# Wubeizhongxinghua/BSSeqConsensusReads

Measured on AMD Instinct MI355X. Metric: duplex families/sec (node) at 1/2/4/8 MI355X; % HBM roofline; speedup vs CPU, higher is better.
Workload: dtype int64 fixed-point log-likelihood sums (2^-20 nats) + fp32 exp; fp64 read-order sums on near ties; u8 nt16 bases / phred quals; 1 GPU; C2 -- configs[1]: 1M-family synthetic WGBS grouped BAM, 2x150bp, Poisson(4) family size, one MI355X; families_per_gpu=1000000, consensus_families_per_gpu=1151121, batches_per_gpu=1, family_order=fgbio TemplateCoordinate runs of one MI, records_per_gpu=8150056, bases_per_gpu=1222508400, small_families=1151121, large_families=0, parallelism=family-sharded x1

## Files before the change

bsseqconsensusreads_amd/csrc/bsdc_kernels.hip:

```cpp
#include <hip/hip_runtime.h>

#include <algorithm>
#include <cmath>
#include <cstdio>
#include <cstdlib>
#include <cstring>
#include <string>

#include "../../include/bsdc.h"
#include "../../include/bsdc_layout.h"

namespace {

constexpr int kWave = 64;
#ifndef SMALL_STAGE_U
#define SMALL_STAGE_U 4
#endif
constexpr int kStageU = SMALL_STAGE_U;
#ifndef LARGE_THREADS
#define LARGE_THREADS 256
#endif
constexpr int kLargeThreads = LARGE_THREADS;
#ifndef LARGE_THREADS_BIG
#define LARGE_THREADS_BIG 512
// ... 566 lines not shown
    }
}
struct OvlDw {
    Ovl4 in;
    uint32_t A0, inm;
    int32_t B0;
    int lo, hi;
};
__device__ __forceinline__ OvlDw ovl_dw_load(const uint8_t *bimg, const uint8_t *qimg, uint32_t xa, uint32_t xb, int ovl,
                                            int d) {
    OvlDw t;
    const int p0 = 4 * d - (int)(xa & 3u);
    t.A0 = (xa & ~3u) + 4u * (uint32_t)d;
    t.B0 = (int32_t)xb + p0;
    t.lo = ::max(-p0, 0);
    t.hi = ::min(ovl - p0, 4);
    t.inm = t.hi > t.lo ? (0xFFFFFFFFu >> (32 - 8 * (t.hi - t.lo))) << (8 * t.lo) : 0u;
    if (t.hi > t.lo) {
        const int32_t Bl = t.B0 + t.lo;
        const uint32_t sh = 8u * (uint32_t)t.lo;
        t.in = Ovl4{lds32(bimg + t.A0), lds_any32(bimg, Bl) << sh, lds32(qimg + t.A0), lds_any32(qimg, Bl) << sh};
    }
    return t;
}
__device__ __forceinline__ void ovl_dw_store(uint8_t *bimg, uint8_t *qimg, const OvlDw &t) {
    if (t.hi <= t.lo) return;
    const Ovl4 o = ovl4_compute_m(t.in, t.inm);
    const bool whole = t.inm == 0xFFFFFFFFu;
    st32(bimg + t.A0, o.x);
    st32(qimg + t.A0, o.qa);
    if (whole && (t.B0 & 3) == 0) {
        st32(bimg + t.B0, o.y);
        st32(qimg + t.B0, o.qb);
    } else if (whole) {
        stu32(bimg + t.B0, o.y);
        stu32(qimg + t.B0, o.qb);
    } else {
        for (int k = t.lo; k < t.hi; k++) {
            bimg[t.B0 + k] = (uint8_t)(o.y >> (8 * k));
            qimg[t.B0 + k] = (uint8_t)(o.qb >> (8 * k));
        }
    }
}
__device__ __forceinline__ void ovl4_store(uint8_t *bimg, uint8_t *qimg, uint32_t ia, uint32_t ib, int rem, const Ovl4 &o) {
    if (rem >= 4) {
        stu32(bimg + ia, o.x);
        stu32(bimg + ib, o.y);
        stu32(qimg + ia, o.qa);
        stu32(qimg + ib, o.qb);
    } else {
        for (int k = 0; k < rem; k++) {
            bimg[ia + k] = (uint8_t)(o.x >> (8 * k));
            bimg[ib + k] = (uint8_t)(o.y >> (8 * k));
            qimg[ia + k] = (uint8_t)(o.qa >> (8 * k));
            qimg[ib + k] = (uint8_t)(o.qb >> (8 * k));
        }
    }
}
__device__ __forceinline__ void overlap4(uint8_t *bimg, uint8_t *qimg, uint32_t ia, uint32_t ib, int rem) {
    ovl4_store(bimg, qimg, ia, ib, rem, ovl4_compute(ovl4_load(bimg, qimg, ia, ib), rem));
}
__device__ __forceinline__ void lookup4(const int32_t *lr2, uint32_t b, uint32_t q, int32_t &D0, int32_t &D1,
                                        int32_t &D2, int32_t &D3) {
    const uint32_t v = (b >> 4) & 0x01010101u;
    const uint32_t lo = __builtin_amdgcn_perm(v, q, 0x05010400u) << 2;
    const uint32_t hi = __builtin_amdgcn_perm(v, q, 0x07030602u) << 2;
    const uint8_t *base = reinterpret_cast<const uint8_t *>(lr2);
    D0 += *reinterpret_cast<const int32_t *>(base + (lo & 0xFFFFu));
    D1 += *reinterpret_cast<const int32_t *>(base + (lo >> 16));
    D2 += *reinterpret_cast<const int32_t *>(base + (hi & 0xFFFFu));
    D3 += *reinterpret_cast<const int32_t *>(base + (hi >> 16));
}
__device__ __forceinline__ void lookup4v(const int32_t *lr2, uint32_t v, uint32_t q, int32_t &D0, int32_t &D1,
                                         int32_t &D2, int32_t &D3) {
    const uint32_t lo = __builtin_amdgcn_perm(v, q, 0x05010400u) << 2;
    const uint32_t hi = __builtin_amdgcn_perm(v, q, 0x07030602u) << 2;
    const uint8_t *base = reinterpret_cast<const uint8_t *>(lr2);
    D0 += *reinterpret_cast<const int32_t *>(base + (lo & 0xFFFFu));
    D1 += *reinterpret_cast<const int32_t *>(base + (lo >> 16));
    D2 += *reinterpret_cast<const int32_t *>(base + (hi & 0xFFFFu));
    D3 += *reinterpret_cast<const int32_t *>(base + (hi >> 16));
}
__device__ __forceinline__ uint32_t onehot01(uint32_t x) {
    const uint32_t r = __builtin_amdgcn_perm(0x00000001u, 0x00018100u, x);
    return r & ~((x + 0x03030303u) >> 4) & 0x01010101u;
}
__device__ __forceinline__ uint32_t bytes_past(int k8, bool reverse) {
    const uint32_t s = (uint32_t)::min(::max(k8, 0), 32);
    return reverse ? (uint32_t)(0xFFFFFFFFull >> s) : (uint32_t)(~0ull << s);
}
__device__ __forceinline__ uint32_t expand80(uint32_t m80) { return m80 | (m80 - (m80 >> 7)); }
__device__ __forceinline__ uint32_t bytes_nonzero(uint32_t x) {
    return expand80((x + 0x7F7F7F7Fu) & 0x80808080u);
}
__device__ __forceinline__ void resolve4(bool ha, bool hb, uint32_t bmA, uint32_t QA, uint32_t bmB, uint32_t QB,
                                         uint32_t qadd, uint32_t &ob, uint32_t &oq, uint32_t *ss) {
    const uint32_t okA = expand80((QA + qadd) & 0x80808080u);
    const uint32_t okB = expand80((QB + qadd) & 0x80808080u);
    const uint32_t bA = (bmA & okA) | (0x0F0F0F0Fu & ~okA), qA = (QA & okA) | (0x02020202u & ~okA);
    const uint32_t bB = (bmB & okB) | (0x0F0F0F0Fu & ~okB), qB = (QB & okB) | (0x02020202u & ~okB);
    ss[0] = bA;
    ss[1] = qA;
    ss[2] = bB;
    ss[3] = qB;
    if (!(ha && hb)) {
        ob = ha ? bA : bB;
        oq = ha ? qA : qB;
        return;
    }
    const uint32_t same = ~bytes_nonzero(bA ^ bB);
    const uint32_t dAB = (qA | 0x80808080u) - qB;
    const uint32_t geA = expand80(dAB & 0x80808080u);
    const uint32_t dBA = (qB | 0x80808080u) - qA;
    const uint32_t ad = ((dAB & geA) | (dBA & ~geA)) & 0x7F7F7F7Fu;
    const uint32_t sum = qA + qB;
    const uint32_t over = expand80((sum + 0x22222222u) & 0x80808080u);
    const uint32_t sum93 = (sum & ~over) | (0x5D5D5D5Du & over);
    const uint32_t ad2 = ad | (0x02020202u & ~bytes_nonzero(ad));
    uint32_t rb = (bA & (same | geA)) | (bB & ~(same | geA));
    uint32_t rq = (sum93 & same) | (ad2 & ~same);
    const uint32_t isN = ((bA + 0x01010101u) | (bB + 0x01010101u)) & 0x10101010u;
    const uint32_t is2 = ~bytes_nonzero(rq ^ 0x02020202u);
    const uint32_t nm = expand80(isN << 3) | is2;
    ob = (rb & ~nm) | (0x0F0F0F0Fu & nm);
    oq = (rq & ~nm) | (0x02020202u & nm);
}
__device__ __forceinline__ uint32_t comp4(uint32_t x) {
    return (__builtin_bitreverse32(__builtin_bswap32(x)) >> 4) & 0x0F0F0F0Fu;
}
template <bool FLAG>
__device__ __forceinline__ void unpack32(uint4 v, uint8_t *dst) {
    const uint32_t w[4] = {v.x, v.y, v.z, v.w};
    uint32_t o[8];
#pragma unroll
    for (int k = 0; k < 4; k++) {
        uint32_t lo = w[k] & 0x0F0F0F0Fu;
        uint32_t hi = (w[k] >> 4) & 0x0F0F0F0Fu;
        if (FLAG) {
            const uint32_t a = w[k], b = w[k] >> 1, c = w[k] >> 2, d = w[k] >> 3;
            const uint32_t ab = a | b, cd = c | d;
            const uint32_t two = (a & b) | (c & d) | (ab & cd);
            const uint32_t vm = (ab | cd) & ~two & 0x11111111u;
            lo |= (vm << 4) & 0x10101010u;
            hi |= vm & 0x10101010u;
        }
        o[2 * k] = __builtin_amdgcn_perm(lo, hi, 0x05010400u);
        o[2 * k + 1] = __builtin_amdgcn_perm(lo, hi, 0x07030602u);
    }
    uint4 *d = reinterpret_cast<uint4 *>(dst);
    d[0] = make_uint4(o[0], o[1], o[2], o[3]);
    d[1] = make_uint4(o[4], o[5], o[6], o[7]);
}

template <bool TAGS>
__device__ __forceinline__ void small_family(const KParams &P, const Tables *T, uint8_t *A, const uint32_t *fams,
                                             int64_t fi, int t) {
    const int32_t *lr2 = T->zero;
    const float *thr = T->thr;
    const uint8_t *qlo = T->qlo;
    const int32_t *dthr = T->dthr;
    const bsdc_family_batch &B = P.B;
    const bool do_convert = P.mode & BSDC_MODE_CONVERT;
    const bool do_extend = P.mode & BSDC_MODE_EXTEND;
    const bool do_vote = P.mode & BSDC_MODE_VOTE;
    const int max_len = B.max_len;
    const int stop = (P.mode >> BSDC_MODE_STOP_SHIFT) & 15;

    const uint4 ent = reinterpret_cast<const uint4 *>(fams)[__builtin_amdgcn_readfirstlane((int)fi)];
    const uint32_t fam = __builtin_amdgcn_readfirstlane(ent.x);
    const uint32_t r0 = __builtin_amdgcn_readfirstlane(ent.y);
    const int n = (int)(__builtin_amdgcn_readfirstlane(ent.z) & 0xFF);
    const uint32_t img = (__builtin_amdgcn_readfirstlane(ent.z) >> 8) * 32u;
    const uint32_t base_g = __builtin_amdgcn_readfirstlane(ent.w);

    const bool has = t < n;
    uint4 rc = make_uint4(0, 0, 0, 0);
    uint2 win = make_uint2(0, 0);
    uint32_t cinfo = 0;
    if (has) {
        rc = reinterpret_cast<const uint4 *>(B.rec)[r0 + t];
        win = reinterpret_cast<const uint2 *>(B.rec_win)[r0 + t];
        cinfo = B.cig_info[r0 + t];
    }
    const int nqc = (int)(img >> 4), nch = nqc + (int)(img >> 5);
    uint8_t *bimg = A;
    uint8_t *qimg = A + img;
    uint32_t qor = 0;
    for (int u = 0; u < ((nqc + 63) >> 6); u++) {
        const int k = t + 64 * u;
        if (k < nqc) glds16(B.qual + base_g + 16u * (uint32_t)k, qimg + 1024 * u);
    }
    auto load_img = [&](int k) {
        uint4 v = make_uint4(0, 0, 0, 0);
        if (k < nch) v = *reinterpret_cast<const uint4 *>(B.seq + (base_g >> 1) + 16 * (uint32_t)(k - nqc));
        return v;
    };
    auto store_img = [&](int k, uint4 v) {
        if (k < nch) unpack32<true>(v, bimg + 32 * (k - nqc));
    };
    auto kmap = [&](int u) {
        const int kb = t + 64 * u;
        return kb < nch - nqc ? nqc + kb : nch;
    };
    uint4 v[kStageU];
#pragma unroll
    for (int u = 0; u < kStageU; u++) v[u] = load_img(kmap(u));

    const uint32_t gslot = rc.x;
    int32_t pos = (int32_t)rc.y;
    const int32_t L = (int32_t)(rc.z & 0xFFFF);
    const uint32_t flag = rc.z >> 16;
    uint32_t link = rc.w;
    const bool conv = has && do_convert && (link & BSDC_LINK_CONVERT);
    const bool cplx = has && (link & BSDC_LINK_COMPLEX);
    if (!cplx) cinfo = 0;
    const uint64_t conv_mask = ballot(conv);
    const int nconv = __builtin_popcountll(conv_mask);
    const int ci = mbcnt(conv_mask);
    int cops = (int)(cinfo & 0xFFFF);
    if (ballot(cops != 0)) {
#pragma unroll
        for (int o = 32; o >= 1; o >>= 1) cops += __shfl_xor(cops, o, kWave);
    }
    const SmallLayout Lo(n, img, nconv, cops, max_len);
    uint8_t *refw = A + Lo.ref;
    const int ws = Lo.ws;
    uint32_t *lc = reinterpret_cast<uint32_t *>(A + Lo.misc);
    uint8_t *convlane = A + Lo.misc + 16;
    uint32_t *convwin = reinterpret_cast<uint32_t *>(A + Lo.lists);
    const uint32_t slot = gslot - base_g;
    if (conv) {
        convwin[ci] = win.x;
        convlane[ci] = (uint8_t)t;
    }
    if (t < 4) lc[t] = 0;
    wave_sync();
    const uint32_t rcn = (uint32_t)P.ref_chunks, rinv = P.ref_chunks_inv;
    const int wtot = nconv * (int)rcn;
    auto load_win = [&](int k) {
        uint4 x = make_uint4(0, 0, 0, 0);
        if (k < wtot) {
            const uint32_t cr = __umulhi((uint32_t)k, rinv), part = (uint32_t)k - cr * rcn;
            x = *reinterpret_cast<const uint4 *>(P.ref + ((convwin[cr] >> 1) & ~15u) + 16 * part);
        }
        return x;
    };
    auto store_win = [&](int k, uint4 x) {
        if (k < wtot) {
            const uint32_t cr = __umulhi((uint32_t)k, rinv), part = (uint32_t)k - cr * rcn;
            unpack32<false>(x, refw + cr * ws + 32 * part);
        }
    };
    uint4 wv[2];
#pragma unroll
    for (int u = 0; u < 2; u++) wv[u] = load_win(t + 64 * u);
    __builtin_amdgcn_s_setprio(0);
#pragma unroll
    for (int u = 0; u < kStageU; u++) store_img(kmap(u), v[u]);
    const int ub = (nch - nqc + 63) >> 6;
    for (int u0 = kStageU; u0 < ub; u0 += kStageU) {
#pragma unroll
        for (int u = 0; u < kStageU; u++) v[u] = load_img(kmap(u0 + u));
#pragma unroll
        for (int u = 0; u < kStageU; u++) store_img(kmap(u0 + u), v[u]);
    }
#pragma unroll
    for (int u = 0; u < 2; u++) store_win(t + 64 * u, wv[u]);
    for (int k0 = 128; k0 < wtot; k0 += 128) {
#pragma unroll
        for (int u = 0; u < 2; u++) wv[u] = load_win(k0 + t + 64 * u);
#pragma unroll
        for (int u = 0; u < 2; u++) store_win(k0 + t + 64 * u, wv[u]);
    }
    __asm__ volatile("s_waitcnt vmcnt(0)" ::: "memory");
    wave_sync();
    for (int k = t; k < nqc; k += 64) {
        const uint4 q = *reinterpret_cast<const uint4 *>(qimg + 16 * k);
        qor |= q.x | q.y | q.z | q.w;
    }
    wave_sync();
    if (stop == 1) return;

    int32_t start = 1, len = L;
    bool rd = false;
    for (int cr0 = 0; cr0 < nconv; cr0 += 4) {
        const int cr = cr0 + (t >> 4);
        const bool act = cr < nconv;
        const int src = act ? convlane[cr] : 0;
        const uint32_t s_slot = (uint32_t)__shfl((int)slot, src, kWave);
        const int32_t s_L = __shfl(L, src, kWave);
        const uint32_t s_win = (uint32_t)__shfl((int)win.x, src, kWave);
        const int32_t s_avail = __shfl((int)win.y, src, kWave);
        bool my_rd = false;
        if (act) {
            const int32_t Lm = s_L + 1;
            const uint32_t wbase = (uint32_t)(cr * ws) + (s_win & 31u);
            for (int j4 = 4 * (t & 15); j4 < Lm; j4 += 64) {
                uint32_t m = lds32(bimg + s_slot + j4);
                const uint32_t mn = lds32(bimg + s_slot + j4 + 4);
                const uint32_t a = wbase + (uint32_t)j4;
                const uint32_t d0 = lds32(refw + (a & ~3u)), d1 = lds32(refw + (a & ~3u) + 4);
                const uint32_t sh = a & 3u;
                uint32_t f0 = alignbyte(d1, d0, sh);
                uint32_t f1 = sh == 3 ? d1 : alignbyte(d1, d0, sh + 1);
                if (j4 + 5 > s_avail) {
#pragma unroll
                    for (int k = 0; k < 4; k++) {
                        if (j4 + k >= s_avail) f0 = (f0 & ~(0xFFu << (8 * k))) | (kN << (8 * k));
                        if (j4 + k + 1 >= s_avail) f1 = (f1 & ~(0xFFu << (8 * k))) | (kN << (8 * k));
                    }
                }
                if (j4 == 0) {
                    const uint32_t r0b = f0 & 0xFFu;
                    m = (m & ~0xFFu) | r0b | ((r0b != 0 && (r0b & (r0b - 1)) == 0) ? 0x10u : 0u);
                }
                const uint32_t m1 = alignbyte(mn, m, 1);
                uint32_t nxt = 0x80808080u;
                const int last = Lm - 1 - j4;
                if (last >= 0 && last < 4) nxt &= ~(0xFFu << (8 * last));
                const uint32_t out = convert4f(m, m1, f0, f1, nxt);
                st32(bimg + s_slot + j4, out);
                if (last >= 0 && last < 4)
                    my_rd = ((out >> (8 * last)) & 0x0F) == kC && ((f1 >> (8 * last)) & 0x0F) == kG;
            }
            if ((t & 15) == 0) qimg[s_slot] = 40;
        }
        const uint64_t bal = ballot(my_rd);
        if (conv && (ci >> 2) == (cr0 >> 2) && ((bal >> (16 * (ci & 3))) & 0xFFFFu)) rd = true;
    }
    if (conv) {
        start = 0;
        len = L + 1 - (rd ? 1 : 0);
        pos = pos - 1 > 0 ? pos - 1 : 0;
    }
    if (!do_convert && has && (link & BSDC_LINK_RD_IN)) rd = true;
    if (rd) link |= kLinkRdDev;
    wave_sync();
    if (stop == 2) return;

    if (do_extend) {
        const int p = (int)((link >> BSDC_LINK_PARTNER_SHIFT) & 3u);
        const uint32_t p_slot = (uint32_t)__shfl((int)slot, p, kWave);
        const int32_t p_start = __shfl(start, p, kWave);
        const int32_t p_len = __shfl(len, p, kWave);
        const bool er = has && (link & BSDC_LINK_EXT_RIGHT);
        const bool el = has && (link & BSDC_LINK_EXT_LEFT) && rd;
        uint32_t b0 = 0, q0 = 0, bl = 0, ql = 0;
        if (er) {
            b0 = bimg[p_slot + p_start];
            q0 = qimg[p_slot + p_start];
        }
        if (el) {
            if (p_len > 0) {
                bl = bimg[p_slot + p_start + p_len - 1];
                ql = qimg[p_slot + p_start + p_len - 1];
            } else {
                bl = bimg[slot + start];
                ql = qimg[slot + start];
            }
        }
        if (er) {
            bimg[slot + start - 1] = (uint8_t)b0;
            qimg[slot + start - 1] = (uint8_t)q0;
            start -= 1;
            len += 1;
            pos -= 1;
        }
        if (el) {
            bimg[slot + start + len] = (uint8_t)bl;
            qimg[slot + start + len] = (uint8_t)ql;
            len += 1;
        }
        wave_sync();
    }

    int32_t reflen = len;
    if (cplx) {
        reflen = (int32_t)(cinfo >> 16) + (conv ? 1 : 0) - ((conv && rd) ? 1 : 0) +
                 ((do_extend && (link & BSDC_LINK_EXT_RIGHT)) ? 1 : 0) +
                 ((do_extend && (link & BSDC_LINK_EXT_LEFT) && rd) ? 1 : 0);
    }

    if (P.mode & BSDC_MODE_DUMP) {
        for (int r = 0; r < n; r++) {
            const uint32_t s_slot = rlu(slot, r), s_g = rlu(gslot, r);
            const int32_t s_start = rl(start, r), s_len = rl(len, r);
            for (int j = t; j < s_len; j += 64) {
                P.O.dump_seq[s_g + j] = bimg[s_slot + s_start + j] & 0x0F;
                P.O.dump_qual[s_g + j] = qimg[s_slot + s_start + j];
            }
        }
        if (has) {
            const uint32_t gi = r0 + t;
            P.O.dump_pos[gi] = pos;
            P.O.dump_len[gi] = (uint16_t)len;
            uint8_t tg = 0;
            if (rd) tg |= 1;
            if (conv) tg |= 2 | 4;
            if (do_extend && (link & BSDC_LINK_EXT_RIGHT)) tg |= 4;
            if (do_extend && (link & BSDC_LINK_EXT_LEFT) && rd) tg |= 8;
            P.O.dump_tags[gi] = tg;
        }
    }
    if (!do_vote || stop == 3) return;

// ... 250 lines not shown
                        const uint32_t q0 = qlo[d >> 16];
                        Qp[side] |= (q0 + (d >= dthr[q0 + 1] ? 1u : 0u)) << (8 * j);
                    }
                }
                uint32_t ob4, oq4, ss[4];
                resolve4(hA, hB, bm[0], Qp[0], bm[1], Qp[1], qadd, ob4, oq4, ss);
                const uint32_t inA = TAGS ? ~bytes_past(8 * (la - c), false) : ~0u;
                const uint32_t inB = TAGS ? ~bytes_past(8 * (lb - c), false) : ~0u;
                const uint32_t slowA = hA ? (bytes_nonzero(multi[0] & 0x7F7F7F7Fu) | negm[0]) & inA : 0u;
                const uint32_t slowB = hB ? (bytes_nonzero(multi[1] & 0x7F7F7F7Fu) | negm[1]) & inB : 0u;
                const uint32_t slow4 = (slowA | slowB) & ~bytes_past(8 * (lv - c), false);
                if (slow4) {
                    const uint32_t useA = hA ? ~slowA : 0u, useB = (hB ? ~slowB : 0u) & ~useA;
                    const uint32_t fb = (ss[0] & useA) | ((ss[2] | 0x10101010u) & useB);
                    const uint32_t fq = (ss[1] & useA) | (ss[3] & useB);
                    ob4 = (ob4 & ~slow4) | (fb & slow4);
                    oq4 = (oq4 & ~slow4) | (fq & slow4);
                }
#pragma unroll
                for (int j = 0; j < 4; j++) {
                    const bool qd = ((slow4 >> (8 * j)) & 0xFFu) != 0;
                    const uint64_t ms = ballot(qd);
                    if (ms == 0) continue;
                    if (qd) sq[nq + mbcnt(ms)] = (uint16_t)((e << 15) | (c + j));
                    nq += __builtin_popcountll(ms);
                }
                if (c < lv) {
                    st32(outb + e * ow + c, ob4);
                    st32(outq + e * ow + c, oq4);
                }
                if (TAGS && c < lv) {
#pragma unroll
                    for (int side = 0; side < 2; side++) {
                        const int s = side == 0 ? sa : sb;
                        if (!(side == 0 ? hA : hB)) continue;
                        const uint32_t n4 = nf[side] + __builtin_bswap32(nr[side]);
                        const int64_t at = (4 * (int64_t)fam + s) * stride + c;
                        *reinterpret_cast<uint32_t *>(P.O.ss_base + at) = ss[2 * side];
                        *reinterpret_cast<uint32_t *>(P.O.ss_qual + at) = ss[2 * side + 1];
                        *reinterpret_cast<uint32_t *>(P.O.ss_depth + at) = n4;
                        *reinterpret_cast<uint32_t *>(P.O.ss_err + at) = 0u;
                    }
                }
            }
        }
        wave_sync();
        if (stop == 7) nq = 0;
        const uint32_t hsm = (hs[0] ? 1u : 0u) | (hs[1] ? 2u : 0u) | (hs[2] ? 4u : 0u) | (hs[3] ? 8u : 0u);
        const int side = t & 1;
        for (int k0 = 0; k0 < 2 * nq && stop != 9; k0 += 64) {
            const int k = (k0 + t) >> 1;
            const bool act = k < nq;
            const uint32_t ent = act ? sq[k] : 0u;
            const int e = (int)(ent >> 15), c = (int)(ent & 0x7FFF);
            const int s = side == 0 ? e : 3 - e;
            const int ns = s == 0 ? cnt[0] : s == 1 ? cnt[1] : s == 2 ? cnt[2] : cnt[3];
            const int os = s == 0 ? off[0] : s == 1 ? off[1] : s == 2 ? off[2] : off[3];
            const bool have = act && ((hsm >> s) & 1u);
            const uint32_t kb = act ? outb[e * ow + c] : 0u, kq = act ? outq[e * ow + c] : 0u;
            uint32_t vb = 0, vq = 0;
            if (have && kq != 0 && (int)((kb >> 4) & 1) == side) {
                vb = kb & 0x0F;
                vq = kq;
            } else if (have) {
                int32_t D0 = 0, D1 = 0, D2 = 0, D3 = 0;
                uint32_t n0 = 0, n1 = 0, n2 = 0, n3 = 0;
                uint32_t seen = 0;
                for (int i = 0; i < ns; i++) {
                    const uint32_t d = dlist[os + i];
                    if (c >= (int)((d >> 16) & 0x7FFF)) continue;
                    const uint32_t idx = (d & 0x80000000u) ? (d & 0xFFFF) - c : (d & 0xFFFF) + c;
                    const uint32_t braw = bimg[idx];
                    seen |= braw;
                    const int32_t v = lr2[(braw >> 4) * 256u + qimg[idx]];
                    const uint32_t bb = (d & 0x80000000u) ? comp_nt16(braw) : (braw & 0x0F);
                    D0 += bb == kA ? v : 0;
                    D1 += bb == kC ? v : 0;
                    D2 += bb == kG ? v : 0;
                    D3 += bb == kT ? v : 0;
                    if (TAGS) {
                        n0 += bb == kA ? 1u : 0u;
                        n1 += bb == kC ? 1u : 0u;
                        n2 += bb == kG ? 1u : 0u;
                        n3 += bb == kT ? 1u : 0u;
                    }
                }
                int best = first_max4(D0, D1, D2, D3);
                if (near_tie(D0, D1, D2, D3, best, ns))
                    best = fp64_pick(SmallDesc{dlist + os}, ns, c, bimg, qimg, P.tab->lnc, P.tab->lne3);
                const SsCall sc = ss_call(D0, D1, D2, D3, best, (seen & 0x10u) != 0, n0, n1, n2, n3, thr, P.qmin);
                vb = sc.base;
                vq = sc.qual;
                if (TAGS) {
                    const int64_t at = (4 * (int64_t)fam + s) * stride + c;
                    P.O.ss_base[at] = (uint8_t)vb;
                    P.O.ss_qual[at] = (uint8_t)vq;
                    P.O.ss_depth[at] = (uint8_t)sc.depth;
                    P.O.ss_err[at] = (uint8_t)sc.err;
                }
            }
            const uint32_t pb = (uint32_t)__shfl_xor((int)vb, 1, kWave), pq = (uint32_t)__shfl_xor((int)vq, 1, kWave);
            if (act && side == 0) {
                const bool ha = (hsm >> e) & 1u, hb = (hsm >> (3 - e)) & 1u;
                uint32_t ob, oq;
                if (ha && hb) {
                    duplex_col(vb, vq, pb, pq, ob, oq);
                } else {
                    ob = ha ? vb : pb;
                    oq = ha ? vq : pq;
                }
                outb[e * ow + c] = (uint8_t)ob;
                outq[e * ow + c] = (uint8_t)oq;
            }
        }
        wave_sync();
        if (stop != 7 && stop != 8) {
            const int e = t >> 5;
            const int ol = e ? olen[1] : olen[0];
            for (int c0 = 8 * (t & 31); c0 < ol; c0 += 256) {
                uint2 bv = *reinterpret_cast<const uint2 *>(outb + e * ow + c0);
                uint2 qv = *reinterpret_cast<const uint2 *>(outq + e * ow + c0);
                const int k8 = 8 * (ol - c0);
                const uint32_t keep0 = ~bytes_past(k8, false), keep1 = ~bytes_past(k8 - 32, false);
                bv.x &= keep0;
                bv.y &= keep1;
                const uint32_t qlo2 = qv.x & keep0, qhi2 = qv.y & keep1;
                const uint32_t t0 = (bv.x << 4) | (bv.x >> 8), t1 = (bv.y << 4) | (bv.y >> 8);
                const uint32_t pk = __builtin_amdgcn_perm(t1, t0, 0x06040200u);
                const int64_t so = (2 * (int64_t)fam + e) * stride;
                *reinterpret_cast<uint32_t *>(P.O.seq + so / 2 + c0 / 2) = pk;
                *reinterpret_cast<uint2 *>(P.O.qual + so + c0) = make_uint2(qlo2, qhi2);
            }
        }
    }
    if (TAGS && t < 4) P.O.ss_len[4 * fam + t] = (uint16_t)(t == 0 ? (hs[0] ? lcs[0] : 0) : t == 1 ? (hs[1] ? lcs[1] : 0)
                                                             : t == 2 ? (hs[2] ? lcs[2] : 0) : (hs[3] ? lcs[3] : 0));
    if (t == 0) {
        uint8_t st = emit ? 1 : 0;
        if (hs[0] || hs[1]) st |= 2;
        if (hs[2] || hs[3]) st |= 4;
        P.O.status[fam] = st;
        P.O.len[2 * fam] = (uint16_t)(emit ? olen[0] : 0);
        P.O.len[2 * fam + 1] = (uint16_t)(emit ? olen[1] : 0);
    }
}

template <bool TAGS>
__global__ __launch_bounds__(kWave *kSmallMaxWaves, kSmallMinWaves) __attribute__((amdgpu_num_sgpr(96))) void k_small(
    KParams P, const uint32_t *fams, int64_t nfams, int32_t arena) {
    extern __shared__ __attribute__((aligned(16))) uint8_t smem[];
    __shared__ __attribute__((aligned(16))) Tables s_tab;
    if (((P.mode >> BSDC_MODE_STOP_SHIFT) & 15) == 15) return;
    __builtin_amdgcn_s_setprio(3);
    load_tables<kTabBytes>(&P.tab->t, reinterpret_cast<uint8_t *>(&s_tab));
    if (((P.mode >> BSDC_MODE_STOP_SHIFT) & 15) == 14) return;
    const int w = threadIdx.x >> 6;
    const int t = threadIdx.x & 63;
    const int64_t fi = (int64_t)blockIdx.x * (blockDim.x >> 6) + w;
    uint8_t *A = smem + kArenaGuard + (size_t)w * (size_t)arena;
    if (fi < nfams) small_family<TAGS>(P, &s_tab, A, fams, fi, t);
}

struct RecMeta {
    int32_t pos;
    int32_t len;
    uint32_t slot;
    int32_t avail;
    int32_t start;
    uint32_t link;
    uint32_t gidx;
    uint32_t win;
    int32_t srclen;
    int32_t reflen;
    uint16_t flag;
    uint8_t rd;
    uint8_t set;
    int32_t in_len;
};
static_assert(sizeof(RecMeta) == bsdc_layout::kRecMetaBytes, "RecMeta layout");


template <int G>
__device__ __forceinline__ int block_sum(int v, int *red) {
#pragma unroll
    for (int o = 32; o >= 1; o >>= 1) v += __shfl_xor(v, o, kWave);
    __syncthreads();
    if ((threadIdx.x & 63) == 0) red[threadIdx.x >> 6] = v;
    __syncthreads();
    int s = 0;
    for (int w = 0; w < G / kWave; w++) s += red[w];
    __syncthreads();
    return s;
}
template <int G>
__device__ __forceinline__ int block_max(int v, int *red) {
#pragma unroll
    for (int o = 32; o >= 1; o >>= 1) v = ::max(v, __shfl_xor(v, o, kWave));
    __syncthreads();
    if ((threadIdx.x & 63) == 0) red[threadIdx.x >> 6] = v;
    __syncthreads();
    int s = red[0];
    for (int w = 1; w < G / kWave; w++) s = ::max(s, red[w]);
    __syncthreads();
    return s;
}

template <int G>
__device__ __forceinline__ void block_sum_max(int a, int b, int *red, int &sum, int &mx) {
#pragma unroll
    for (int o = 32; o >= 1; o >>= 1) {
        a += __shfl_xor(a, o, kWave);
        b = ::max(b, __shfl_xor(b, o, kWave));
    }
    if ((threadIdx.x & 63) == 0) {
        red[threadIdx.x >> 6] = a;
        red[G / kWave + (threadIdx.x >> 6)] = b;
    }
    __syncthreads();
    sum = 0;
    mx = red[G / kWave];
    for (int w = 0; w < G / kWave; w++) {
        sum += red[w];
        mx = ::max(mx, red[G / kWave + w]);
    }
}

template <int G, bool TAGS>
__device__ void large_emit(const KParams &P, uint32_t fam, const int *cnt, const int *lcv, const uint8_t *ssb,
                           const uint8_t *ssq, int ssw, bool tag_rows) {
    const int tt = threadIdx.x;
    bool hs[4];
    for (int s = 0; s < 4; s++) hs[s] = cnt[s] > 0 && lcv[s] > 0;
    const bool emit = (hs[0] || hs[3]) && (hs[1] || hs[2]);
    const int32_t stride = P.O.stride;
    int olen[2];
    for (int e = 0; e < 2; e++) {
        const int sa = e == 0 ? 0 : 1, sb2 = e == 0 ? 3 : 2;
        olen[e] = (hs[sa] && hs[sb2]) ? ::min(lcv[sa], lcv[sb2]) : hs[sa] ? lcv[sa] : hs[sb2] ? lcv[sb2] : 0;
    }
    if (emit) {
        for (int e = 0; e < 2; e++) {
            const int sa = e == 0 ? 0 : 1, sb2 = e == 0 ? 3 : 2;
            const int64_t so = (2 * (int64_t)fam + e) * stride;
            const int npair = (olen[e] + 1) >> 1;
            for (int k = tt; k < npair; k += G) {
                uint32_t ob[2] = {0, 0}, oq[2] = {0, 0};
                for (int h = 0; h < 2; h++) {
                    const int col = 2 * k + h;
                    if (col >= olen[e]) break;
                    if (hs[sa] && hs[sb2]) {
                        duplex_col(ssb[sa * ssw + col], ssq[sa * ssw + col], ssb[sb2 * ssw + col], ssq[sb2 * ssw + col],
                                   ob[h], oq[h]);
                    } else {
                        const int s1 = hs[sa] ? sa : sb2;
                        ob[h] = ssb[s1 * ssw + col];
                        oq[h] = ssq[s1 * ssw + col];
                    }
                }
                P.O.seq[so / 2 + k] = (uint8_t)((ob[0] << 4) | ob[1]);
                P.O.qual[so + 2 * k] = (uint8_t)oq[0];
                if (2 * k + 1 < olen[e]) P.O.qual[so + 2 * k + 1] = (uint8_t)oq[1];
            }
        }
    }
    if (TAGS && tag_rows) {
        for (int s = 0; s < 4; s++) {
            const int ls = hs[s] ? lcv[s] : 0;
            const int64_t row = (4 * (int64_t)fam + s) * stride;
            for (int c = tt; c < ls; c += G) {
                P.O.ss_base[row + c] = ssb[s * ssw + c];
                P.O.ss_qual[row + c] = ssq[s * ssw + c];
            }
        }
        if (tt < 4) P.O.ss_len[4 * fam + tt] = (uint16_t)(hs[tt] ? lcv[tt] : 0);
    }
    if (tt == 0) {
        uint8_t st = emit ? 1 : 0;
        if (hs[0] || hs[1]) st |= 2;
        if (hs[2] || hs[3]) st |= 4;
        P.O.status[fam] = st;
        P.O.len[2 * fam] = (uint16_t)(emit ? olen[0] : 0);
        P.O.len[2 * fam + 1] = (uint16_t)(emit ? olen[1] : 0);
    }
}


template <bool SEL>
__device__ __forceinline__ int pick4(const int (&a)[4], int s) {
    if constexpr (SEL)
        return s == 0 ? a[0] : s == 1 ? a[1] : s == 2 ? a[2] : a[3];
    else
        return a[s];
}
__device__ __forceinline__ bool multi_base(uint32_t m) {
    return ((m & 0xFFu) != 0) + ((m & 0xFF00u) != 0) + ((m & 0xFF0000u) != 0) + ((m & 0xFF000000u) != 0) > 1;
}
struct PartSums {
    int32_t *head;
    uint4 *sum;
    uint32_t *cnt;
    int32_t pitch;
    __device__ __forceinline__ PartSums(const KParams &P) {
        uint8_t *b = P.O.scratch + P.B.split_partial_off;
        const int64_t np = P.B.n_split_parts;
        pitch = P.O.stride;
        head = reinterpret_cast<int32_t *>(b);
        sum = reinterpret_cast<uint4 *>(b + round16(32 * np));
        cnt = reinterpret_cast<uint32_t *>(b + round16(32 * np) + 16 * 4 * np * (int64_t)pitch);
        one = reinterpret_cast<int32_t *>(b + round16(32 * np) + 20 * 4 * np * (int64_t)pitch);
    }
    int32_t *one;
    __device__ __forceinline__ uint8_t *orb(int64_t at) const { return reinterpret_cast<uint8_t *>(cnt) + at; }
    __device__ __forceinline__ int64_t at(int64_t part, int s, int col) const { return (4 * part + s) * (int64_t)pitch + col; }
// ... 1429 lines not shown
```

Measured before the change: 351.0 million families/s.

## Overlap lookup-table staging with family record and image loads in small kernel

The small-family kernel no longer stages the lookup tables to LDS with a blocking load and barrier before any family work starts. It issues the table loads into registers, loads the family entry through a scalar constant-address pointer, and starts the record and image global loads. Only then does it write the tables to LDS and synchronize. Dead waves now take part in the barrier and return afterwards, and setup that depends on the records (conversion ballot, cigar ops, layout) is moved after the barrier. This hides table-load latency behind the first family loads, but it holds more registers and the layout is now built with nconv and cops set to zero.

```diff
diff --git a/bsseqconsensusreads_amd/csrc/bsdc_kernels.hip b/bsseqconsensusreads_amd/csrc/bsdc_kernels.hip
--- a/bsseqconsensusreads_amd/csrc/bsdc_kernels.hip
+++ b/bsseqconsensusreads_amd/csrc/bsdc_kernels.hip
@@ -742,9 +742,9 @@
     d[1] = make_uint4(o[4], o[5], o[6], o[7]);
 }
 
-template <bool TAGS>
-__device__ __forceinline__ void small_family(const KParams &P, const Tables *T, uint8_t *A, const uint32_t *fams,
-                                             int64_t fi, int t) {
+template <bool TAGS, class Publish>
+__device__ __forceinline__ void small_family(const KParams &P, const Tables *T, uint8_t *A, const uint4 ent, const bool live,
+                                             int t, Publish &&publish) {
     const int32_t *lr2 = T->zero;
     const float *thr = T->thr;
     const uint8_t *qlo = T->qlo;
@@ -756,11 +756,11 @@
     const int max_len = B.max_len;
     const int stop = (P.mode >> BSDC_MODE_STOP_SHIFT) & 15;
 
-    const uint4 ent = reinterpret_cast<const uint4 *>(fams)[__builtin_amdgcn_readfirstlane((int)fi)];
     const uint32_t fam = __builtin_amdgcn_readfirstlane(ent.x);
     const uint32_t r0 = __builtin_amdgcn_readfirstlane(ent.y);
-    const int n = (int)(__builtin_amdgcn_readfirstlane(ent.z) & 0xFF);
-    const uint32_t img = (__builtin_amdgcn_readfirstlane(ent.z) >> 8) * 32u;
+    const uint32_t entz = live ? __builtin_amdgcn_readfirstlane(ent.z) : 0u;
+    const int n = (int)(entz & 0xFF);
+    const uint32_t img = (entz >> 8) * 32u;
     const uint32_t base_g = __builtin_amdgcn_readfirstlane(ent.w);
 
     const bool has = t < n;
@@ -795,37 +795,22 @@
     uint4 v[kStageU];
 #pragma unroll
     for (int u = 0; u < kStageU; u++) v[u] = load_img(kmap(u));
-
-    const uint32_t gslot = rc.x;
-    int32_t pos = (int32_t)rc.y;
-    const int32_t L = (int32_t)(rc.z & 0xFFFF);
-    const uint32_t flag = rc.z >> 16;
-    uint32_t link = rc.w;
-    const bool conv = has && do_convert && (link & BSDC_LINK_CONVERT);
-    const bool cplx = has && (link & BSDC_LINK_COMPLEX);
-    if (!cplx) cinfo = 0;
-    const uint64_t conv_mask = ballot(conv);
-    const int nconv = __builtin_popcountll(conv_mask);
-    const int ci = mbcnt(conv_mask);
-    int cops = (int)(cinfo & 0xFFFF);
-    if (ballot(cops != 0)) {
-#pragma unroll
-        for (int o = 32; o >= 1; o >>= 1) cops += __shfl_xor(cops, o, kWave);
-    }
-    const SmallLayout Lo(n, img, nconv, cops, max_len);
+    publish();
+    if (stop == 14) __asm__ volatile("s_waitcnt vmcnt(0)" ::: "memory");
+    if (stop == 14 || !live) return;
+
+    const SmallLayout Lo(n, img, 0, 0, max_len);
     uint8_t *refw = A + Lo.ref;
     const int ws = Lo.ws;
     uint32_t *lc = reinterpret_cast<uint32_t *>(A + Lo.misc);
     uint8_t *convlane = A + Lo.misc + 16;
     uint32_t *convwin = reinterpret_cast<uint32_t *>(A + Lo.lists);
-    const uint32_t slot = gslot - base_g;
-    if (conv) {
-        convwin[ci] = win.x;
-        convlane[ci] = (uint8_t)t;
-    }
-    if (t < 4) lc[t] = 0;
-    wave_sync();
     const uint32_t rcn = (uint32_t)P.ref_chunks, rinv = P.ref_chunks_inv;
+    uint32_t link = rc.w;
+    const bool conv = has && do_convert && (link & BSDC_LINK_CONVERT);
+    const uint64_t conv_mask = ballot(conv);
+    const int nconv = __builtin_popcountll(conv_mask);
+    const int ci = mbcnt(conv_mask);
     const int wtot = nconv * (int)rcn;
     auto load_win = [&](int k) {
         uint4 x = make_uint4(0, 0, 0, 0);
@@ -841,6 +826,24 @@
             unpack32<false>(x, refw + cr * ws + 32 * part);
         }
     };
+    const uint32_t gslot = rc.x;
+    int32_t pos = (int32_t)rc.y;
+    const int32_t L = (int32_t)(rc.z & 0xFFFF);
+    const uint32_t flag = rc.z >> 16;
+    const bool cplx = has && (link & BSDC_LINK_COMPLEX);
+    if (!cplx) cinfo = 0;
+    int cops = (int)(cinfo & 0xFFFF);
+    if (ballot(cops != 0)) {
+#pragma unroll
+        for (int o = 32; o >= 1; o >>= 1) cops += __shfl_xor(cops, o, kWave);
+    }
+    const uint32_t slot = gslot - base_g;
+    if (conv) {
+        convwin[ci] = win.x;
+        convlane[ci] = (uint8_t)t;
+    }
+    if (t < 4) lc[t] = 0;
+    wave_sync();
     uint4 wv[2];
 #pragma unroll
     for (int u = 0; u < 2; u++) wv[u] = load_win(t + 64 * u);
@@ -1397,13 +1400,29 @@
     __shared__ __attribute__((aligned(16))) Tables s_tab;
     if (((P.mode >> BSDC_MODE_STOP_SHIFT) & 15) == 15) return;
     __builtin_amdgcn_s_setprio(3);
-    load_tables<kTabBytes>(&P.tab->t, reinterpret_cast<uint8_t *>(&s_tab));
-    if (((P.mode >> BSDC_MODE_STOP_SHIFT) & 15) == 14) return;
     const int w = threadIdx.x >> 6;
     const int t = threadIdx.x & 63;
     const int64_t fi = (int64_t)blockIdx.x * (blockDim.x >> 6) + w;
+    const int fiu = __builtin_amdgcn_readfirstlane((int)fi);
+    const bool live = fiu < nfams;
+    typedef uint32_t u32x4 __attribute__((ext_vector_type(4)));
+    typedef const __attribute__((address_space(4))) u32x4 *EntPtr;
+    const u32x4 e4 = *(EntPtr)(uintptr_t)(fams + 4 * (size_t)(live ? fiu : (int)nfams - 1));
+    const uint4 ent = make_uint4(e4.x, e4.y, e4.z, e4.w);
+    static_assert(kTabBytes / 16 <= 2 * 4 * kWave, "two rounds of table chunks");
+    const uint4 *tsrc = reinterpret_cast<const uint4 *>(&P.tab->t);
+    const int i0 = (int)threadIdx.x, i1 = (int)(threadIdx.x + blockDim.x);
+    uint4 tv0 = make_uint4(0, 0, 0, 0), tv1 = tv0;
+    if (i0 < kTabBytes / 16) tv0 = tsrc[i0];
+    if (i1 < kTabBytes / 16) tv1 = tsrc[i1];
+    auto publish = [&]() {
+        uint4 *td = reinterpret_cast<uint4 *>(&s_tab);
+        if (i0 < kTabBytes / 16) td[i0] = tv0;
+        if (i1 < kTabBytes / 16) td[i1] = tv1;
+        __syncthreads();
+    };
     uint8_t *A = smem + kArenaGuard + (size_t)w * (size_t)arena;
-    if (fi < nfams) small_family<TAGS>(P, &s_tab, A, fams, fi, t);
+    small_family<TAGS>(P, &s_tab, A, ent, live, t, publish);
 }
 
 struct RecMeta {
```

New measurement: 350.9 million families/s. About the same (-0.0%).
